# MP-ReID/mp-reid

Measured on AMD Instinct MI355X. Metric: gallery images/s encode + distmat+rerank ms, 20k×20k; mAP/Rank-1 parity, higher is better.
Workload: dtype f16 pairs hi+lo (3 MFMA products per multiply-add, f32-grade), f32 acc; distmat f32 exact; 1 GPU; Market-1501 configs[1]: do_inference ViT-B/16 3368q+15913g/GPU, no rerank; HBM-resident loader; encoder_batch=508, encoder_precision=split, encoder_streams=2, rerank=False, distance_mode=exact

## Files before the change

mp-reid_amd/csrc/gemm_f16.h:

```cpp
#pragma once
#include "common.h"

typedef _Float16 f16x8 __attribute__((ext_vector_type(8)));
typedef float f32x4 __attribute__((ext_vector_type(4)));

constexpr int GBM = 128, GBN = 128, GBK = 64;
constexpr int G_TILE_BYTES = GBM * GBK * 2;
constexpr int G_STAGE_BYTES = 2 * G_TILE_BYTES;
constexpr int G_LDS_BYTES = 2 * G_STAGE_BYTES;
constexpr int BBM = 256, BBN = 256, BBK = 32, B_NSTAGE = 4;
constexpr int B_PART_BYTES = BBM * BBK * 2;
constexpr int B_STAGE_BYTES = 2 * B_PART_BYTES;
constexpr int B_LDS_BYTES = B_NSTAGE * B_STAGE_BYTES;
constexpr int B_LDS_TOTAL = B_LDS_BYTES + 8 * 4096;
constexpr int PBM = 256, PBN = 128, PBK = 32, P_NSTAGE = 3;
constexpr int P_A_BYTES = PBM * PBK * 2;
constexpr int P_B_BYTES = PBN * PBK * 2;
constexpr int P_STAGE_BYTES = P_A_BYTES + P_B_BYTES;
constexpr int P_RING_BYTES = P_NSTAGE * P_STAGE_BYTES;
constexpr int P_LDS_BYTES = P_RING_BYTES + 4 * 1024;

enum GemmEpi {
    GE_F32 = 0,
    GE_BIAS_F16 = 1,
    GE_BIAS_RES = 2,
    GE_BIAS_GELU = 3,
    GE_PATCH = 4,
    GE_EUCLID = 5,
    GE_COSINE = 6,
    GE_BIAS_RELU = 7,
    GE_BIAS_ADD_RELU = 8,
    GE_CAND = 9,
    GE_S_BIAS_F32 = 10,
    GE_S_BIAS_RES = 11,
    GE_S_BIAS_GELU = 12,
    GE_S_PATCH = 13,
    GE_S_BIAS_RELU_PAIR = 14
    , GE_S_BIAS_RES_PAIR = 15
};
constexpr bool gemm_epi_is_split(int epi) { return epi >= GE_S_BIAS_F32 && epi <= GE_S_BIAS_RES_PAIR; }
constexpr bool gemm_epi_has_big(int epi) {
    return epi == GE_F32 || epi == GE_BIAS_F16 || epi == GE_BIAS_RES || epi == GE_BIAS_GELU || epi == GE_EUCLID || epi == GE_PATCH ||
           epi == GE_BIAS_RELU || epi == GE_BIAS_ADD_RELU || epi == GE_CAND || gemm_epi_is_split(epi);
}

struct GemmArgs {
    const _Float16 *A;
    const _Float16 *W;
    int M, N, K;
    int kseg;
    float oscale;
    void *out;
    int64_t ldo;
    const float *bias;
    const float *aux;
    const float *aux2;
    int m_valid, n_valid;
    int P, L;
    const _Float16 *identity;
    const float *rscale;
    const float *cscale;
    const float *tlo, *thi;
    unsigned *cnt_lo, *cnt_hi;
    uint2 *list_lo, *list_hi;
    int cap_lo, cap_hi, sym;
    int stagger;
    int stagger_mode;
    int walk;
    int pair_c;
    _Float16 *pair_out;
    int relu_x;
    unsigned long long *stamps;
};

int launch_gemm_f16(const GemmArgs &a, int epi, hipStream_t stream);
```

mp-reid_amd/csrc/gemm_f16.hip:

```cpp
#include <algorithm>
#include <cstdlib>
#include <type_traits>

#include "gemm_plan.h"

typedef __attribute__((address_space(3))) void lds_ptr_t;
typedef const __attribute__((address_space(1))) void glb_ptr_t;

__device__ __forceinline__ void dma16(const void *gsrc, unsigned char *lds_dst_wave_base) {
    __builtin_amdgcn_global_load_lds((glb_ptr_t *)gsrc, (lds_ptr_t *)lds_dst_wave_base, 16, 0, 0);
}

__device__ __forceinline__ unsigned lds_addr(const void *p) {
    return (unsigned)(uintptr_t)(const __attribute__((address_space(3))) void *)p;
}
__device__ __forceinline__ void dma16_sv(uint64_t sbase, unsigned voff, unsigned lds_dst) {
    unsigned keep;
    asm volatile("s_mov_b32 %0, m0\n\t"
                 "s_mov_b32 m0, %3\n\t"
                 "s_nop 0\n\t"
                 "global_load_lds_dwordx4 %2, %1 nt\n\t"
                 "s_mov_b32 m0, %0"
                 : "=&s"(keep)
                 : "s"(sbase), "v"(voff), "s"(lds_dst)
                 : "memory");
}
__device__ __forceinline__ void store16_sv(uint64_t sbase, unsigned voff, const f32x4 &v) {
    asm volatile("global_store_dwordx4 %0, %1, %2\n\ts_nop 1" ::"v"(voff), "v"(v), "s"(sbase) : "memory");
}
typedef unsigned u32x2 __attribute__((ext_vector_type(2)));
__device__ __forceinline__ void store8_sv(uint64_t sbase, unsigned voff, const u32x2 &v) {
    asm volatile("global_store_dwordx2 %0, %1, %2\n\ts_nop 1" ::"v"(voff), "v"(v), "s"(sbase) : "memory");
}
__device__ __forceinline__ void store16_nt_sv(uint64_t sbase, unsigned voff, const f32x4 &v) {
    asm volatile("global_store_dwordx4 %0, %1, %2 nt\n\ts_nop 1" ::"v"(voff), "v"(v), "s"(sbase) : "memory");
}
template <int F>
__device__ __forceinline__ void store16_flav_sv(uint64_t sbase, unsigned voff, const f32x4 &v) {
    if constexpr (F == 1) asm volatile("global_store_dwordx4 %0, %1, %2\n\ts_nop 1" ::"v"(voff), "v"(v), "s"(sbase) : "memory");
    else if constexpr (F == 2) asm volatile("global_store_dwordx4 %0, %1, %2 sc1\n\ts_nop 1" ::"v"(voff), "v"(v), "s"(sbase) : "memory");
    else if constexpr (F == 3) asm volatile("global_store_dwordx4 %0, %1, %2 sc0 sc1\n\ts_nop 1" ::"v"(voff), "v"(v), "s"(sbase) : "memory");
    else if constexpr (F == 4) asm volatile("global_store_dwordx4 %0, %1, %2 sc0 sc1 nt\n\ts_nop 1" ::"v"(voff), "v"(v), "s"(sbase) : "memory");
    else if constexpr (F == 5) asm volatile("global_store_dwordx4 %0, %1, %2 sc0\n\ts_nop 1" ::"v"(voff), "v"(v), "s"(sbase) : "memory");
    else store16_nt_sv(sbase, voff, v);
}

__device__ __forceinline__ void wait_vmcnt(int n) {
    switch (n) {
    case 12: asm volatile("s_waitcnt vmcnt(12)" ::: "memory"); break;
    case 16: asm volatile("s_waitcnt vmcnt(16)" ::: "memory"); break;
    case 20: asm volatile("s_waitcnt vmcnt(20)" ::: "memory"); break;
    case 24: asm volatile("s_waitcnt vmcnt(24)" ::: "memory"); break;
    case 36: asm volatile("s_waitcnt vmcnt(36)" ::: "memory"); break;
    case 40: asm volatile("s_waitcnt vmcnt(40)" ::: "memory"); break;
    case 44: asm volatile("s_waitcnt vmcnt(44)" ::: "memory"); break;
    case 48: asm volatile("s_waitcnt vmcnt(48)" ::: "memory"); break;
    default: asm volatile("s_waitcnt vmcnt(0)" ::: "memory"); break;
    }
}

__device__ __forceinline__ float quick_gelu(float h) {
    return h * __builtin_amdgcn_rcpf(1.0f + __builtin_amdgcn_exp2f(-1.702f * 1.44269504088896340736f * h));
}

typedef unsigned u32x4_t __attribute__((ext_vector_type(4)));
typedef float f32x4_t __attribute__((ext_vector_type(4)));
__device__ __forceinline__ void store_nt(void *p, const uint4 &v) {
    const u32x4_t nv = {v.x, v.y, v.z, v.w};
    __builtin_nontemporal_store(nv, reinterpret_cast<u32x4_t *>(p));
}
__device__ __forceinline__ void store_nt(float *p, const float4 &v) {
    const f32x4_t nv = {v.x, v.y, v.z, v.w};
    __builtin_nontemporal_store(nv, reinterpret_cast<f32x4_t *>(p));
}

template <int EPI>
__global__ __launch_bounds__(256, 2) void gemm_f16_kernel(GemmArgs g, int tiles_m, int tiles_n) {
    extern __shared__ __attribute__((aligned(16))) unsigned char smem[];

    int tm, tn;
    tile_coords(xcd_remap(blockIdx.x, gridDim.x), tiles_m, tiles_n, 8, tm, tn);
    const int m0 = tm * GBM, n0 = tn * GBN;
    const int tid = threadIdx.x, lane = tid & 63;
    const int wave = __builtin_amdgcn_readfirstlane(tid >> 6);
    const int wm = wave >> 1, wn = wave & 1;
    const int K = g.K;
    constexpr bool SPLIT = gemm_epi_is_split(EPI);
    const int nseg = SPLIT ? g.kseg / GBK : 0;

    const int srow = lane >> 3;
    const int gchunk = (lane & 7) ^ srow;
    const _Float16 *a_src = g.A + (int64_t)(m0 + wave * 32 + srow) * K + gchunk * 8;
    const _Float16 *b_src = g.W + (int64_t)(n0 + wave * 32 + srow) * K + gchunk * 8;
    auto stage = [&](int s, int kt) {
        unsigned char *abase = smem + s * G_STAGE_BYTES + wave * 4096;
        unsigned char *bbase = abase + G_TILE_BYTES;
        const int koff = kt * GBK;
#pragma unroll
        for (int t = 0; t < 4; ++t) {
            dma16(a_src + (int64_t)t * 8 * K + koff, abase + t * 1024);
            dma16(b_src + (int64_t)t * 8 * K + koff, bbase + t * 1024);
        }
    };

    const int frow = lane & 15, fq = lane >> 4;
    const int a_row_off = (wm * 64 + frow) * 128;
    const int b_row_off = (wn * 64 + frow) * 128;
    int ksw[2];
    ksw[0] = ((0 + fq) ^ (lane & 7)) << 4;
    ksw[1] = ((4 + fq) ^ (lane & 7)) << 4;

    f32x4 acc[4][4];
#pragma unroll
    for (int i = 0; i < 4; ++i)
#pragma unroll
        for (int j = 0; j < 4; ++j) acc[i][j] = f32x4{0.f, 0.f, 0.f, 0.f};

    auto compute = [&](int s) {
        const unsigned char *at = smem + s * G_STAGE_BYTES;
        const unsigned char *bt = at + G_TILE_BYTES;
#pragma unroll
        for (int ks = 0; ks < 2; ++ks) {
            f16x8 af[4], bf[4];
#pragma unroll
            for (int i = 0; i < 4; ++i) af[i] = *reinterpret_cast<const f16x8 *>(at + a_row_off + i * 2048 + ksw[ks]);
#pragma unroll
            for (int j = 0; j < 4; ++j) bf[j] = *reinterpret_cast<const f16x8 *>(bt + b_row_off + j * 2048 + ksw[ks]);
#pragma unroll
            for (int i = 0; i < 4; ++i)
#pragma unroll
                for (int j = 0; j < 4; ++j)
                    acc[i][j] = __builtin_amdgcn_mfma_f32_16x16x32_f16(af[i], bf[j], acc[i][j], 0, 0, 0);
        }
    };

    if constexpr (SPLIT) {
        for (int kb = 0; kb < nseg; ++kb) {
            if (kb) __syncthreads();
            {
                unsigned char *abase = smem + wave * 4096;
#pragma unroll
                for (int part = 0; part < 2; ++part) {
                    const int koff = part * g.kseg + kb * GBK;
#pragma unroll
                    for (int t = 0; t < 4; ++t) {
                        dma16(a_src + (int64_t)t * 8 * K + koff, abase + part * G_STAGE_BYTES + t * 1024);
                        dma16(b_src + (int64_t)t * 8 * K + koff, abase + part * G_STAGE_BYTES + G_TILE_BYTES + t * 1024);
                    }
                }
            }
            __syncthreads();
            const unsigned char *ah = smem, *bh = smem + G_TILE_BYTES, *al = smem + G_STAGE_BYTES,
                                *bl = smem + G_STAGE_BYTES + G_TILE_BYTES;
#pragma unroll
            for (int ks = 0; ks < 2; ++ks) {
                f16x8 afh[4], afl[4], bfh[4], bfl[4];
#pragma unroll
                for (int i = 0; i < 4; ++i) {
                    afh[i] = *reinterpret_cast<const f16x8 *>(ah + a_row_off + i * 2048 + ksw[ks]);
                    afl[i] = *reinterpret_cast<const f16x8 *>(al + a_row_off + i * 2048 + ksw[ks]);
                }
#pragma unroll
                for (int j = 0; j < 4; ++j) {
                    bfh[j] = *reinterpret_cast<const f16x8 *>(bh + b_row_off + j * 2048 + ksw[ks]);
                    bfl[j] = *reinterpret_cast<const f16x8 *>(bl + b_row_off + j * 2048 + ksw[ks]);
                }
#pragma unroll
                for (int i = 0; i < 4; ++i)
#pragma unroll
                    for (int j = 0; j < 4; ++j) {
                        acc[i][j] = __builtin_amdgcn_mfma_f32_16x16x32_f16(afh[i], bfh[j], acc[i][j], 0, 0, 0);
                        acc[i][j] = __builtin_amdgcn_mfma_f32_16x16x32_f16(afl[i], bfh[j], acc[i][j], 0, 0, 0);
                        acc[i][j] = __builtin_amdgcn_mfma_f32_16x16x32_f16(afh[i], bfl[j], acc[i][j], 0, 0, 0);
                    }
// ... 154 lines not shown
                    }
                    o[0] = x.x + o[0];
                    o[1] = x.y + o[1];
                    o[2] = x.z + o[2];
                    o[3] = x.w + o[3];
                }
                *reinterpret_cast<float4 *>(dst) = make_float4(o[0], o[1], o[2], o[3]);
                if constexpr (EPI == GE_S_BIAS_RES_PAIR) {
                    typedef _Float16 h4p __attribute__((ext_vector_type(4)));
                    h4p hi, lo;
                    {
                        const float y[4] = {o[0] < 0.f ? 0.f : o[0], o[1] < 0.f ? 0.f : o[1], o[2] < 0.f ? 0.f : o[2],
                                            o[3] < 0.f ? 0.f : o[3]};
                        split_pairs<4>(y, hi, lo);
                    }
                    _Float16 *po = g.pair_out + m * 2 * g.pair_c + nbase + c4;
                    *reinterpret_cast<h4p *>(po) = hi;
                    *reinterpret_cast<h4p *>(po + g.pair_c) = lo;
                }
            }
            __syncthreads();
        }
    } else if constexpr (EPI == GE_BIAS_RES || EPI == GE_EUCLID || EPI == GE_F32) {
        __syncthreads();
        float *wreg = reinterpret_cast<float *>(smem) + wave * (32 * 68);
        float *outp = reinterpret_cast<float *>(g.out);
        const bool vec_ok = (g.ldo % 4 == 0) && ((reinterpret_cast<uintptr_t>(outp) & 15) == 0);
#pragma unroll
        for (int half = 0; half < 2; ++half) {
#pragma unroll
            for (int ii = 0; ii < 2; ++ii)
#pragma unroll
                for (int j = 0; j < 4; ++j)
#pragma unroll
                    for (int r = 0; r < 4; ++r)
                        wreg[(ii * 16 + fq * 4 + r) * 68 + j * 16 + frow] = acc[half * 2 + ii][j][r];
            __syncthreads();
            const int mbase = m0 + wm * 64 + half * 32, nbase = n0 + wn * 64;
            if (vec_ok) {
                const int c4 = (lane & 15) * 4;
                float4 bias4 = make_float4(0.f, 0.f, 0.f, 0.f), bn4 = bias4;
                if (EPI == GE_BIAS_RES) bias4 = *reinterpret_cast<const float4 *>(g.bias + nbase + c4);
                if (EPI == GE_EUCLID) {
                    bn4.x = (nbase + c4 + 0 < g.n_valid) ? g.aux2[nbase + c4 + 0] : 0.f;
                    bn4.y = (nbase + c4 + 1 < g.n_valid) ? g.aux2[nbase + c4 + 1] : 0.f;
                    bn4.z = (nbase + c4 + 2 < g.n_valid) ? g.aux2[nbase + c4 + 2] : 0.f;
                    bn4.w = (nbase + c4 + 3 < g.n_valid) ? g.aux2[nbase + c4 + 3] : 0.f;
                }
#pragma unroll
                for (int it = 0; it < 8; ++it) {
                    const int lr = it * 4 + (lane >> 4);
                    const int m = mbase + lr;
                    const float4 a = *reinterpret_cast<const float4 *>(wreg + lr * 68 + c4);
                    float *dst = outp + (int64_t)m * g.ldo + nbase + c4;
                    if (EPI == GE_F32) {
                        *reinterpret_cast<float4 *>(dst) = a;
                    } else if (EPI == GE_BIAS_RES) {
                        float4 x = *reinterpret_cast<const float4 *>(dst);
                        x.x = x.x + (a.x + bias4.x);
                        x.y = x.y + (a.y + bias4.y);
                        x.z = x.z + (a.z + bias4.z);
                        x.w = x.w + (a.w + bias4.w);
                        *reinterpret_cast<float4 *>(dst) = x;
                    } else {
                        if (m < g.m_valid) {
                            const float am = g.aux[m];
                            float4 o, s4 = make_float4(1.f, 1.f, 1.f, 1.f);
                            if (g.rscale) {
                                const float rs = g.rscale[m];
                                s4 = make_float4(rs * g.cscale[nbase + c4 + 0], rs * g.cscale[nbase + c4 + 1],
                                                 rs * g.cscale[nbase + c4 + 2], rs * g.cscale[nbase + c4 + 3]);
                            }
                            o.x = fmaf(-2.0f, a.x * s4.x, am + bn4.x);
                            o.y = fmaf(-2.0f, a.y * s4.y, am + bn4.y);
                            o.z = fmaf(-2.0f, a.z * s4.z, am + bn4.z);
                            o.w = fmaf(-2.0f, a.w * s4.w, am + bn4.w);
                            if (nbase + c4 + 3 < g.n_valid) {
                                *reinterpret_cast<float4 *>(dst) = o;
                            } else {
                                if (nbase + c4 + 0 < g.n_valid) dst[0] = o.x;
                                if (nbase + c4 + 1 < g.n_valid) dst[1] = o.y;
                                if (nbase + c4 + 2 < g.n_valid) dst[2] = o.z;
                            }
                        }
                    }
                }
            } else {
                const int n = nbase + lane;
                float bias = 0.f, bnv = 0.f;
                if (EPI == GE_BIAS_RES) bias = g.bias[n];
                if (EPI == GE_EUCLID) bnv = (n < g.n_valid) ? g.aux2[n] : 0.f;
#pragma unroll 4
                for (int lr = 0; lr < 32; ++lr) {
                    const int m = mbase + lr;
                    const float a = wreg[lr * 68 + lane];
                    float *dst = outp + (int64_t)m * g.ldo + n;
                    if (EPI == GE_F32) {
                        *dst = a;
                    } else if (EPI == GE_BIAS_RES) {
                        *dst = *dst + (a + bias);
                    } else if (m < g.m_valid && n < g.n_valid) {
                        const float sc = g.rscale ? g.rscale[m] * g.cscale[n] : 1.0f;
                        *dst = fmaf(-2.0f, a * sc, g.aux[m] + bnv);
                    }
                }
            }
            __syncthreads();
        }
    } else {
#pragma unroll
        for (int j = 0; j < 4; ++j) {
            const int n = n0 + wn * 64 + j * 16 + frow;
            float bnv = 0.f;
            if (EPI == GE_COSINE) bnv = (n < g.n_valid) ? g.aux2[n] : 0.f;
#pragma unroll
            for (int i = 0; i < 4; ++i)
#pragma unroll
                for (int r = 0; r < 4; ++r) {
                    const int m = m0 + wm * 64 + i * 16 + fq * 4 + r;
                    const float a = (EPI == GE_S_PATCH) ? acc[i][j][r] * g.oscale : acc[i][j][r];
                    if (EPI == GE_PATCH || EPI == GE_S_PATCH) {
                        if (m < g.m_valid) {
                            const int b = m / g.P, p = m - b * g.P;
                            reinterpret_cast<float *>(g.out)[((int64_t)b * g.L + 1 + p) * g.ldo + n] =
                                a + g.aux[(int64_t)(1 + p) * g.N + n];
                        }
                    } else if (EPI == GE_COSINE) {
                        if (m < g.m_valid && n < g.n_valid) {
                            const float sc = g.rscale ? g.rscale[m] * g.cscale[n] : 1.0f;
                            float c = (a * sc) * __fdiv_rn(1.0f, g.aux[m] * bnv);
                            const float lo = (float)(-1.0 + 0.00001), hi = (float)(1.0 - 0.00001);
                            c = c < lo ? lo : (c > hi ? hi : c);
                            reinterpret_cast<float *>(g.out)[(int64_t)m * g.ldo + n] = acosf(c);
                        }
                    }
                }
        }
    }
}


template <int EPI, int DBG = 0, bool SYM = false>
__global__ __launch_bounds__(512) void gemm_f16_big_kernel(GemmArgs g, int tiles_m, int tiles_n) {
    extern __shared__ __attribute__((aligned(16))) unsigned char smem[];
    const int tid = threadIdx.x, lane = tid & 63;
    const int wave = __builtin_amdgcn_readfirstlane(tid >> 6);
    const int wr = wave >> 2, wc = wave & 3;
    const int K = g.K;
    constexpr bool SPLIT = gemm_epi_is_split(EPI);
    constexpr bool SYM_STORE = (EPI == GE_EUCLID) && SYM;
    constexpr bool SYM_EPI = (EPI == GE_CAND) || SYM_STORE;
    const int nseg = SPLIT ? g.kseg / BBK : 0;
    const int nst = SPLIT ? 3 * nseg : K / BBK;
    auto koff_a = [&](int st) -> int {
        if constexpr (!SPLIT) return st * BBK;
        const int r = st / 3, sidx = st - 3 * r;
        return sidx == 0 ? r * BBK : (sidx == 1 ? g.kseg + r * BBK : -1);
    };
    auto koff_b = [&](int st) -> int {
        if constexpr (!SPLIT) return st * BBK;
        const int r = st / 3, sidx = st - 3 * r;
        return sidx == 0 ? r * BBK : (sidx == 2 ? g.kseg + r * BBK : -1);
    };

    const int ntiles = tiles_m * tiles_n;
    const int nb = (int)gridDim.x;
    const int GR = ((g.walk & 7) == 3 || (g.walk & 8)) ? 4 : ((g.walk & 7) == 4 ? 16 : 8);
    const bool colfast = (g.walk & 7) == 1;
    const int ngroups = (tiles_m + GR - 1) / GR;
    const bool owned = (nb % 8 == 0) && (tiles_m % (8 * GR) == 0 || (ngroups >= 24 && !(g.walk & 16) && !(SYM_EPI && g.sym)));
    const bool blocked = !owned && (nb % 64 == 0) && ntiles >= nb;
    const int xcd = (int)(blockIdx.x & 7), per_xcd = nb >> 3, per_group = GR * tiles_n;
    const int bc_w = per_xcd >> 3;
    const int nbc = blocked ? (tiles_n + bc_w - 1) / bc_w : 1, nbr = (tiles_m + 7) >> 3;
    const bool symc = SYM_EPI && blocked && g.sym != 0;
    int pos = (owned || symc) ? (int)(blockIdx.x >> 3) : (blocked ? 0 : (int)blockIdx.x);
    const int pos_step = (owned || symc) ? per_xcd : (blocked ? 1 : nb);
    int sy_p = 0, sy_cum = 0;
    auto sym_tile_at = [&](int k) -> int {
        for (;;) {
            int b = sy_p * 8 + xcd, br = 0, bcol = 0;
            for (;; ++br) {
                if (br >= nbr) return -1;
                int fb = (br * 8 - bc_w + 1 + bc_w - 1) / bc_w;
                fb = fb < 0 ? 0 : fb;
                const int cnt = nbc - fb;
                if (cnt > 0 && b < cnt) {
                    bcol = fb + b;
                    break;
                }
                b -= cnt > 0 ? cnt : 0;
            }
            const int c_lo = bcol * bc_w, c_hi = min(tiles_n, c_lo + bc_w);
            int cnt = 0;
            for (int r = 0; r < 8; ++r) {
                const int tm = br * 8 + r;
                if (tm < tiles_m) cnt += max(0, c_hi - max(tm, c_lo));
            }
            if (k < sy_cum + cnt) {
                int want = k - sy_cum;
                for (int sl = 0; sl < 8 * bc_w; ++sl) {
                    const int tm = br * 8 + (sl & 7), tn = c_lo + (sl >> 3);
                    if (tm < tiles_m && tn < tiles_n && tn >= tm && want-- == 0) return tm * tiles_n + tn;
                }
            }
            sy_cum += cnt;
            ++sy_p;
        }
    };
    auto tile_at_raw = [&](int p) -> int {
        if (blocked) {
            int b = p * 8 + xcd, br, bcol;
            if (SYM_EPI && g.sym) {
                br = 0;
                for (;; ++br) {
                    if (br >= nbr) return -1;
                    int fb = (br * 8 - bc_w + 1 + bc_w - 1) / bc_w;
                    fb = fb < 0 ? 0 : fb;
                    const int cnt = nbc - fb;
                    if (cnt > 0 && b < cnt) {
                        bcol = fb + b;
                        break;
                    }
                    b -= cnt > 0 ? cnt : 0;
                }
            } else {
                br = b / nbc;
                bcol = b - br * nbc;
            }
            if (br >= nbr) return -1;
            const int slot = (int)(blockIdx.x >> 3);
            const int tm = br * 8 + (slot & 7), tn = bcol * bc_w + (slot >> 3);
            if (SYM_EPI && g.sym && tn < tm) return -2;
            return (tm < tiles_m && tn < tiles_n) ? tm * tiles_n + tn : -2;
        }
        if (!owned) {
            if (p >= ntiles) return -1;
            if (SYM_EPI && g.sym) {
                int tm, tn;
                tile_coords((unsigned)p, tiles_m, tiles_n, 8, tm, tn);
                if (tn < tm) return -2;
            }
            return p;
        }
        const int grp = xcd + 8 * (p / per_group);
        if (grp >= ngroups) return -1;
        const int within = p % per_group;
        const int wrow = colfast ? within / tiles_n : within % GR, wcol = colfast ? within % tiles_n : within / GR;
        if (grp * GR + wrow >= tiles_m) return -2;
        if (SYM_EPI && g.sym && wcol < grp * GR + wrow) return -2;
        return (grp * GR + wrow) * tiles_n + wcol;
    };
    auto tile_at = [&](int &p) -> int {
        if constexpr (SYM_EPI) {
            if (symc) return sym_tile_at(p);
        }
        int t = tile_at_raw(p);
        while (t == -2) {
            p += pos_step;
            t = tile_at_raw(p);
        }
        return t;
    };

    const int drow = lane >> 2;
    const int dchunk = (lane & 3) ^ (((drow >> 3) & 1) * 3);
    const _Float16 *a_src = nullptr, *b_src = nullptr;
    int m0 = 0, n0 = 0;
    auto set_tile = [&](int tile) {
        int tm, tn;
        if (owned || blocked) {
            tm = tile / tiles_n;
            tn = tile - tm * tiles_n;
        } else {
            tile_coords((unsigned)tile, tiles_m, tiles_n, 8, tm, tn);
        }
        m0 = tm * BBM;
        n0 = tn * BBN;
        const int ma = (DBG == 64) ? (tm & 1) * BBM : m0, na = (DBG == 64) ? (tn & 1) * BBN : n0;
        a_src = g.A + (int64_t)(ma + wave * 32 + drow) * K + dchunk * 8;
        b_src = g.W + (int64_t)(na + wave * 32 + drow) * K + dchunk * 8;
    };
    auto dma_stage = [&](int st) {
        unsigned char *abase = smem + (st & (B_NSTAGE - 1)) * B_STAGE_BYTES + wave * 2048;
        unsigned char *bbase = abase + B_PART_BYTES;
        const int koff = koff_a(st), koffb = koff_b(st);
        if (!SPLIT || koff >= 0) {
            dma16(a_src + koff, abase);
            dma16(a_src + (int64_t)16 * K + koff, abase + 1024);
        }
        if (!SPLIT || koffb >= 0) {
            dma16(b_src + koffb, bbase);
            dma16(b_src + (int64_t)16 * K + koffb, bbase + 1024);
        }
    };
    constexpr bool PAIR = !SPLIT && !(DBG & 16);
    auto dma_pair = [&](int st) {
        unsigned char *a0 = smem + (st & (B_NSTAGE - 1)) * B_STAGE_BYTES + wave * 2048;
        unsigned char *a1 = smem + ((st + 1) & (B_NSTAGE - 1)) * B_STAGE_BYTES + wave * 2048;
        const int k0 = st * BBK, k1 = k0 + BBK;
        dma16(a_src + k0, a0);
        dma16(a_src + k1, a1);
        dma16(a_src + (int64_t)16 * K + k0, a0 + 1024);
        dma16(a_src + (int64_t)16 * K + k1, a1 + 1024);
        dma16(b_src + k0, a0 + B_PART_BYTES);
        dma16(b_src + k1, a1 + B_PART_BYTES);
        dma16(b_src + (int64_t)16 * K + k0, a0 + B_PART_BYTES + 1024);
        dma16(b_src + (int64_t)16 * K + k1, a1 + B_PART_BYTES + 1024);
    };
    auto dma_prologue = [&]() {
        if constexpr (PAIR) {
            dma_pair(0);
            if (2 < nst) dma_pair(2);
        } else {
            dma_stage(0);
            if (1 < nst) dma_stage(1);
            if (2 < nst) dma_stage(2);
        }
    };

    const int frow = lane & 15, fq = lane >> 4;
    const int fsw = (fq ^ (((lane >> 3) & 1) * 3)) << 4;
    const int a_off = (wr * 128 + frow) * 64 + fsw;
    const int b_off = B_PART_BYTES + (wc * 64 + frow) * 64 + fsw;
    auto load_frags = [&](int st, f16x8 (&fa)[8], f16x8 (&fb)[4]) {
        const unsigned char *sb = smem + (st & (B_NSTAGE - 1)) * B_STAGE_BYTES;
#pragma unroll
        for (int j = 0; j < 4; ++j) fb[j] = *reinterpret_cast<const f16x8 *>(sb + b_off + j * 1024);
#pragma unroll
        for (int i = 0; i < 8; ++i) fa[i] = *reinterpret_cast<const f16x8 *>(sb + a_off + i * 1024);
    };

    constexpr int CL_CAP = 336;
    int cl_n = 0;
    unsigned *cl_row = reinterpret_cast<unsigned *>(smem + B_LDS_BYTES + wave * 4096);
    unsigned *cl_col = cl_row + CL_CAP;
    unsigned *cl_d = cl_col + CL_CAP;
    auto cl_flush = [&]() {
        if constexpr (EPI == GE_CAND) {
            __builtin_amdgcn_fence(__ATOMIC_RELEASE, "wavefront");
            __builtin_amdgcn_wave_barrier();
            __builtin_amdgcn_fence(__ATOMIC_ACQUIRE, "wavefront");
            for (int e = lane; e < cl_n; e += 64) {
                const unsigned rw = cl_row[e], cw = cl_col[e], dv = cl_d[e];
                const unsigned fl = rw >> 28, row = rw & 0x0fffffffu;
                if (fl & 1u) {
                    const unsigned p = atomicAdd(&g.cnt_lo[row], 1u);
                    if (p < (unsigned)g.cap_lo) g.list_lo[(size_t)row * g.cap_lo + p] = make_uint2(cw, dv);
                }
                if (fl & 2u) {
                    const unsigned p = atomicAdd(&g.cnt_hi[row], 1u);
                    if (p < (unsigned)g.cap_hi) g.list_hi[(size_t)row * g.cap_hi + p] = make_uint2(cw, dv);
                }
                if (fl & 4u) {
                    const unsigned p = atomicAdd(&g.cnt_lo[cw], 1u);
                    if (p < (unsigned)g.cap_lo) g.list_lo[(size_t)cw * g.cap_lo + p] = make_uint2(row, dv);
                }
                if (fl & 8u) {
                    const unsigned p = atomicAdd(&g.cnt_hi[cw], 1u);
                    if (p < (unsigned)g.cap_hi) g.list_hi[(size_t)cw * g.cap_hi + p] = make_uint2(row, dv);
                }
            }
            __builtin_amdgcn_wave_barrier();
            cl_n = 0;
        }
    };

    int tile = tile_at(pos);
    if (tile < 0) return;
    if (g.stagger > 0) {
        const unsigned long long t0 = __builtin_amdgcn_s_memrealtime();
        const unsigned long long wait = g.stagger_mode ? (unsigned long long)g.stagger * ((blockIdx.x >> 3) & 7u) / 8u
                                                       : (unsigned long long)g.stagger * (blockIdx.x & 255u) / 256u;
        while (__builtin_amdgcn_s_memrealtime() - t0 < wait) __builtin_amdgcn_s_sleep(32);
    }
    set_tile(tile);
    dma_prologue();
    [[maybe_unused]] int stamp_tile = 0;
    for (;;) {
    f32x4 acc[8][4];
#pragma unroll
    for (int i = 0; i < 8; ++i)
#pragma unroll
        for (int j = 0; j < 4; ++j) acc[i][j] = f32x4{0.f, 0.f, 0.f, 0.f};

    if constexpr (SPLIT) asm volatile("s_waitcnt vmcnt(4)\n\ts_barrier" ::: "memory");
    else if constexpr (PAIR) {
        if (nst > 2) asm volatile("s_waitcnt vmcnt(8)\n\ts_barrier" ::: "memory");
        else asm volatile("s_waitcnt vmcnt(0)\n\ts_barrier" ::: "memory");
    } else if (nst > 2) asm volatile("s_waitcnt vmcnt(8)\n\ts_barrier" ::: "memory");
    else asm volatile("s_waitcnt vmcnt(4)\n\ts_barrier" ::: "memory");

    auto stamp = [&](int which) {
        if constexpr ((DBG & 32) != 0) {
            if (g.stamps && tid == 0 && stamp_tile < 32)
                g.stamps[((size_t)blockIdx.x * 32 + stamp_tile) * 8 + which] = __builtin_amdgcn_s_memrealtime();
        }
    };
    stamp(0);
    f16x8 fa0[8], fb0[4], fa1[8], fb1[4];
    load_frags(0, fa0, fb0);

    auto mfma32 = [&](f16x8 (&fa)[8], f16x8 (&fb)[4]) {
#pragma unroll
        for (int i = 0; i < 8; ++i)
#pragma unroll
            for (int j = 0; j < 4; ++j)
                acc[i][j] = __builtin_amdgcn_mfma_f32_16x16x32_f16(fa[i], fb[j], acc[i][j], 0, 0, 0);
    };
    auto step_steady = [&](auto ODD_, int t, f16x8 (&fa)[8], f16x8 (&fb)[4], f16x8 (&na)[8], f16x8 (&nb)[4]) {
        constexpr bool ODD = decltype(ODD_)::value != 0;
        constexpr bool ISSUE = !PAIR || ODD;
        if constexpr (!PAIR) asm volatile("s_waitcnt vmcnt(4)\n\ts_barrier" ::: "memory");
        else if constexpr (ODD) asm volatile("s_waitcnt vmcnt(1) lgkmcnt(0)\n\ts_barrier" ::: "memory");
        else asm volatile("s_waitcnt vmcnt(8)\n\ts_barrier" ::: "memory");
        unsigned char *dbase = smem + ((t + 3) & (B_NSTAGE - 1)) * B_STAGE_BYTES + wave * 2048;
        unsigned char *dbase2 = smem + ((t + 4) & (B_NSTAGE - 1)) * B_STAGE_BYTES + wave * 2048;
        const unsigned char *sb = smem + ((t + 1) & (B_NSTAGE - 1)) * B_STAGE_BYTES;
        const int koff = koff_a(t + 3), koffb = koff_b(t + 3);
#define MPREID_FRAG_B(j) nb[j] = *reinterpret_cast<const f16x8 *>(sb + b_off + (j) * 1024)
#define MPREID_FRAG_A(i) na[i] = *reinterpret_cast<const f16x8 *>(sb + a_off + (i) * 1024)
#define MPREID_MFMA_ROWS(i0)                                                                             \
    _Pragma("unroll") for (int ii = (i0); ii < (i0) + 2; ++ii) _Pragma("unroll") for (int j = 0; j < 4; ++j) { \
        if constexpr (!(DBG & 2))                                                                        \
            acc[ii][j] = __builtin_amdgcn_mfma_f32_16x16x32_f16(fa[ii], fb[j], acc[ii][j], 0, 0, 0);       \
        else                                                                                             \
            asm volatile("" ::"v"(fa[ii]), "v"(fb[j]));                                                  \
    }
        if constexpr (!(DBG & 1) && ISSUE) {
            dma16(a_src + koff, dbase);
            if constexpr (PAIR) dma16(a_src + koff + BBK, dbase2);
        }
        if constexpr (!(DBG & 4)) { MPREID_FRAG_B(0); MPREID_FRAG_B(1); MPREID_FRAG_B(2); }
        MPREID_MFMA_ROWS(0);
        __builtin_amdgcn_sched_barrier(0);
        if constexpr (!(DBG & 1) && ISSUE) {
            dma16(a_src + (int64_t)16 * K + koff, dbase + 1024);
            if constexpr (PAIR) dma16(a_src + (int64_t)16 * K + koff + BBK, dbase2 + 1024);
        }
        if constexpr (!(DBG & 4)) { MPREID_FRAG_B(3); MPREID_FRAG_A(0); MPREID_FRAG_A(1); }
        MPREID_MFMA_ROWS(2);
        __builtin_amdgcn_sched_barrier(0);
        if constexpr (!(DBG & 1) && ISSUE) {
            dma16(b_src + koffb, dbase + B_PART_BYTES);
            if constexpr (PAIR) dma16(b_src + koffb + BBK, dbase2 + B_PART_BYTES);
        }
        if constexpr (!(DBG & 4)) { MPREID_FRAG_A(2); MPREID_FRAG_A(3); MPREID_FRAG_A(4); }
        MPREID_MFMA_ROWS(4);
        __builtin_amdgcn_sched_barrier(0);
        if constexpr (!(DBG & 1) && ISSUE) {
            dma16(b_src + (int64_t)16 * K + koffb, dbase + B_PART_BYTES + 1024);
            if constexpr (PAIR) dma16(b_src + (int64_t)16 * K + koffb + BBK, dbase2 + B_PART_BYTES + 1024);
        }
        if constexpr (!(DBG & 4)) { MPREID_FRAG_A(5); MPREID_FRAG_A(6); MPREID_FRAG_A(7); }
        MPREID_MFMA_ROWS(6);
        __builtin_amdgcn_sched_barrier(0);
#undef MPREID_FRAG_A
#undef MPREID_FRAG_B
#undef MPREID_MFMA_ROWS
    };
    auto step_tail = [&](int t, f16x8 (&fa)[8], f16x8 (&fb)[4], f16x8 (&na)[8], f16x8 (&nb)[4]) {
        if (t + 1 < nst) {
            if constexpr (PAIR) {
                if (!(t & 1) && t + 3 < nst) asm volatile("s_waitcnt vmcnt(8)\n\ts_barrier" ::: "memory");
                else asm volatile("s_waitcnt vmcnt(0)\n\ts_barrier" ::: "memory");
            } else {
                if (t + 2 < nst) asm volatile("s_waitcnt vmcnt(4)\n\ts_barrier" ::: "memory");
                else asm volatile("s_waitcnt vmcnt(0)\n\ts_barrier" ::: "memory");
                if (t + 3 < nst) dma_stage(t + 3);
            }
            load_frags(t + 1, na, nb);
        }
        mfma32(fa, fb);
    };
    if constexpr (SPLIT) {
        auto sstep = [&](auto S_, auto TAIL_, int t) {
            constexpr int S = decltype(S_)::value;
            constexpr bool TAIL = decltype(TAIL_)::value;
            constexpr int s0 = S % 3;
            constexpr bool ldA = s0 != 1, ldB = s0 != 0;
            constexpr bool dmA = s0 != 2, dmB = s0 != 1;
            f16x8 (&fa)[8] = (S & 1) ? fa1 : fa0;
            f16x8 (&fb)[4] = (s0 == 2) ? fb1 : fb0;
            f16x8 (&na)[8] = (S < 3) ? fa1 : fa0;
            f16x8 (&nb)[4] = (s0 == 1) ? fb1 : fb0;
            constexpr bool more1 = !TAIL || S < 5, more3 = !TAIL || S < 3;
            if constexpr (more1) {
                if constexpr (TAIL && S >= 4) asm volatile("s_waitcnt vmcnt(0)\n\ts_barrier" ::: "memory");
                else if constexpr (s0 == 1) asm volatile("s_waitcnt vmcnt(4)\n\ts_barrier" ::: "memory");
                else asm volatile("s_waitcnt vmcnt(2)\n\ts_barrier" ::: "memory");
            }
            unsigned char *dbase = smem + ((t + 3) & (B_NSTAGE - 1)) * B_STAGE_BYTES + wave * 2048;
            const unsigned char *sb = smem + ((t + 1) & (B_NSTAGE - 1)) * B_STAGE_BYTES;
            const int r3 = (t + 3) / 3;
            const int koff = (s0 == 1 ? g.kseg : 0) + r3 * BBK, koffb = (s0 == 2 ? g.kseg : 0) + r3 * BBK;
            auto piece = [&](int q) {
                if (!more3) return;
                if (dmA && q < 2) dma16(a_src + (int64_t)(q * 16) * K + koff, dbase + q * 1024);
                else if (dmB && q - (dmA ? 2 : 0) >= 0 && q - (dmA ? 2 : 0) < 2)
                    dma16(b_src + (int64_t)((q - (dmA ? 2 : 0)) * 16) * K + koffb, dbase + B_PART_BYTES + (q - (dmA ? 2 : 0)) * 1024);
            };
            auto rd_a = [&](int i) { if (more1) na[i] = *reinterpret_cast<const f16x8 *>(sb + a_off + i * 1024); };
            auto rd_b = [&](int j) { if (more1) nb[j] = *reinterpret_cast<const f16x8 *>(sb + b_off + j * 1024); };
#pragma unroll
            for (int gq = 0; gq < 4; ++gq) {
                piece(gq);
                if constexpr (ldA && ldB) {
                    if (gq == 0) { rd_b(0); rd_b(1); rd_b(2); }
                    if (gq == 1) { rd_b(3); rd_a(0); rd_a(1); }
                    if (gq == 2) { rd_a(2); rd_a(3); rd_a(4); }
                    if (gq == 3) { rd_a(5); rd_a(6); rd_a(7); }
                } else if constexpr (ldA) {
                    rd_a(2 * gq);
                    rd_a(2 * gq + 1);
                } else {
                    rd_b(gq);
                }
#pragma unroll
                for (int ii = 2 * gq; ii < 2 * gq + 2; ++ii)
#pragma unroll
                    for (int j = 0; j < 4; ++j)
                        acc[ii][j] = __builtin_amdgcn_mfma_f32_16x16x32_f16(fa[ii], fb[j], acc[ii][j], 0, 0, 0);
                __builtin_amdgcn_sched_barrier(0);
            }
        };
        using std::integral_constant;
        int t = 0;
        for (; t + 6 < nst; t += 6) {
            sstep(integral_constant<int, 0>{}, integral_constant<bool, false>{}, t);
            sstep(integral_constant<int, 1>{}, integral_constant<bool, false>{}, t + 1);
            sstep(integral_constant<int, 2>{}, integral_constant<bool, false>{}, t + 2);
            sstep(integral_constant<int, 3>{}, integral_constant<bool, false>{}, t + 3);
            sstep(integral_constant<int, 4>{}, integral_constant<bool, false>{}, t + 4);
            sstep(integral_constant<int, 5>{}, integral_constant<bool, false>{}, t + 5);
        }
        sstep(integral_constant<int, 0>{}, integral_constant<bool, true>{}, t);
        sstep(integral_constant<int, 1>{}, integral_constant<bool, true>{}, t + 1);
        sstep(integral_constant<int, 2>{}, integral_constant<bool, true>{}, t + 2);
        sstep(integral_constant<int, 3>{}, integral_constant<bool, true>{}, t + 3);
        sstep(integral_constant<int, 4>{}, integral_constant<bool, true>{}, t + 4);
        sstep(integral_constant<int, 5>{}, integral_constant<bool, true>{}, t + 5);
    } else {
    int t = 0;
    for (; t + 4 < nst; t += 2) {
        step_steady(std::integral_constant<int, 0>{}, t, fa0, fb0, fa1, fb1);
        step_steady(std::integral_constant<int, 1>{}, t + 1, fa1, fb1, fa0, fb0);
    }
    for (; t < nst; t += 2) {
        step_tail(t, fa0, fb0, fa1, fb1);
        step_tail(t + 1, fa1, fb1, fa0, fb0);
    }
    }

    __syncthreads();
    stamp(1);
    const int cur_m0 = m0, cur_n0 = n0;
    pos += pos_step;
    const int next_tile = tile_at(pos);
    unsigned char *patch = smem + B_LDS_BYTES;
    if constexpr (DBG & 8) {
#pragma unroll
        for (int i = 0; i < 8; ++i)
#pragma unroll
            for (int j = 0; j < 4; ++j) asm volatile("" ::"v"(acc[i][j]));
    } else if constexpr (EPI == GE_CAND) {
        const bool mirror = g.sym != 0 && cur_m0 != cur_n0;
        float *tp = reinterpret_cast<float *>(smem + wave * 16384);
        const int rb = cur_m0 + wr * 128, cb = cur_n0 + wc * 64;
        const float NEG = -__builtin_huge_valf(), POS = __builtin_huge_valf();
        float *rt = tp + 1024;
        float *ct = rt + 384;
        {
            const float a0 = g.aux[rb + lane], a1 = g.aux[rb + 64 + lane];
            const float l0 = g.tlo[rb + lane], l1 = g.tlo[rb + 64 + lane];
            const float h0 = g.thi[rb + lane], h1 = g.thi[rb + 64 + lane];
            const int c = cb + lane;
            const bool cv = c < g.n_valid;
            const float cn = cv ? g.aux2[c] : 0.f;
            const float cl = (mirror && cv) ? g.tlo[c] : NEG, chh = (mirror && cv) ? g.thi[c] : POS;
            rt[lane] = a0; rt[64 + lane] = a1;
            rt[128 + lane] = l0; rt[192 + lane] = l1;
            rt[256 + lane] = h0; rt[320 + lane] = h1;
            ct[lane] = cn; ct[64 + lane] = cl; ct[128 + lane] = chh;
        }
        __builtin_amdgcn_fence(__ATOMIC_RELEASE, "wavefront");
        __builtin_amdgcn_wave_barrier();
        __builtin_amdgcn_fence(__ATOMIC_ACQUIRE, "wavefront");
        float bnv[4], tlc[4], thc[4];
        unsigned cvm = 0u;
#pragma unroll
        for (int j = 0; j < 4; ++j) {
            const int cl_ = j * 16 + frow;
            cvm |= (cb + cl_ < g.n_valid) ? (0xfu << (4 * j)) : 0u;
            bnv[j] = ct[cl_];
            tlc[j] = ct[64 + cl_];
            thc[j] = ct[128 + cl_];
        }
#pragma unroll
        for (int i = 0; i < 8; ++i) {
            const int rl = i * 16 + fq * 4;
            const int r0 = rb + rl;
            const float4 an4 = *reinterpret_cast<const float4 *>(rt + rl);
            const float4 tl4 = *reinterpret_cast<const float4 *>(rt + 128 + rl);
            const float4 th4 = *reinterpret_cast<const float4 *>(rt + 256 + rl);
            const float anr[4] = {an4.x, an4.y, an4.z, an4.w}, tlr[4] = {tl4.x, tl4.y, tl4.z, tl4.w},
                        thr[4] = {th4.x, th4.y, th4.z, th4.w};
            unsigned rvm = 0u;
#pragma unroll
            for (int r = 0; r < 4; ++r) rvm |= (r0 + r < g.m_valid) ? (0x1111u << r) : 0u;
            unsigned hit = 0u;
#pragma unroll
            for (int j = 0; j < 4; ++j)
#pragma unroll
                for (int r = 0; r < 4; ++r) {
                    const float a = acc[i][j][r];
                    tp[(fq * 4 + r) * 64 + j * 16 + frow] = a;
                    const float d = fmaf(-2.0f, a, anr[r] + bnv[j]);
                    const bool h = (d <= tlr[r]) | (d >= thr[r]) | (d <= tlc[j]) | (d >= thc[j]);
                    hit |= h ? (1u << (j * 4 + r)) : 0u;
                }
            hit &= cvm & rvm;
            __builtin_amdgcn_fence(__ATOMIC_RELEASE, "wavefront");
            __builtin_amdgcn_wave_barrier();
            __builtin_amdgcn_fence(__ATOMIC_ACQUIRE, "wavefront");
            unsigned long long bal = __ballot(hit != 0u);
            if (g.stagger & 2) bal = 0;
            while (bal) {
                const int add = __popcll(bal);
                if (cl_n + add > CL_CAP) cl_flush();
                if (hit) {
                    const int e = __ffs((int)hit) - 1;
                    hit &= hit - 1u;
                    const int j = e >> 2, r = e & 3;
                    const float a = tp[(fq * 4 + r) * 64 + j * 16 + frow];
                    const float anx = r == 0 ? anr[0] : (r == 1 ? anr[1] : (r == 2 ? anr[2] : anr[3]));
                    const float tlx = r == 0 ? tlr[0] : (r == 1 ? tlr[1] : (r == 2 ? tlr[2] : tlr[3]));
                    const float thx = r == 0 ? thr[0] : (r == 1 ? thr[1] : (r == 2 ? thr[2] : thr[3]));
                    const float bnx = j == 0 ? bnv[0] : (j == 1 ? bnv[1] : (j == 2 ? bnv[2] : bnv[3]));
                    const float tcx = j == 0 ? tlc[0] : (j == 1 ? tlc[1] : (j == 2 ? tlc[2] : tlc[3]));
                    const float hcx = j == 0 ? thc[0] : (j == 1 ? thc[1] : (j == 2 ? thc[2] : thc[3]));
                    const float d = fmaf(-2.0f, a, anx + bnx);
                    const unsigned fl = (d <= tlx ? 1u : 0u) | (d >= thx ? 2u : 0u) | (d <= tcx ? 4u : 0u) | (d >= hcx ? 8u : 0u);
                    const int p = cl_n + __popcll(bal & ((1ull << lane) - 1ull));
                    cl_row[p] = (unsigned)(r0 + r) | (fl << 28);
                    cl_col[p] = (unsigned)(cb + j * 16 + frow);
                    cl_d[p] = __float_as_uint(d);
                }
                cl_n += add;
                bal = __ballot(hit != 0u);
            }
            __builtin_amdgcn_wave_barrier();
        }
        if (next_tile < 0) cl_flush();
        asm volatile("s_barrier" ::: "memory");
    } else if constexpr (EPI == GE_BIAS_F16 || EPI == GE_BIAS_GELU || EPI == GE_BIAS_RELU) {
        _Float16 *wreg = reinterpret_cast<_Float16 *>(patch + wave * 4096);
        _Float16 *out = reinterpret_cast<_Float16 *>(g.out);
        float bias[4];
#pragma unroll
        for (int j = 0; j < 4; ++j) bias[j] = g.bias[cur_n0 + wc * 64 + j * 16 + frow];
#pragma unroll
        for (int i = 0; i < 8; ++i) {
#pragma unroll
            for (int j = 0; j < 4; ++j)
#pragma unroll
                for (int r = 0; r < 4; ++r) {
                    float v = acc[i][j][r] + bias[j];
                    if (EPI == GE_BIAS_GELU) v = quick_gelu(v);
                    if (EPI == GE_BIAS_RELU) v = v < 0.f ? 0.f : v;
                    wreg[(fq * 4 + r) * 72 + j * 16 + frow] = (_Float16)v;
                }
            __builtin_amdgcn_fence(__ATOMIC_RELEASE, "wavefront");
            __builtin_amdgcn_wave_barrier();
            __builtin_amdgcn_fence(__ATOMIC_ACQUIRE, "wavefront");
#pragma unroll
            for (int it = 0; it < 2; ++it) {
                const int lr = it * 8 + (lane >> 3), ch = lane & 7;
                const uint4 v = *reinterpret_cast<const uint4 *>(wreg + lr * 72 + ch * 8);
                _Float16 *dsth = out + (int64_t)(cur_m0 + wr * 128 + i * 16 + lr) * g.ldo + cur_n0 + wc * 64 + ch * 8;
                if (EPI == GE_BIAS_RELU) *reinterpret_cast<uint4 *>(dsth) = v;
                else store_nt(dsth, v);
            }
            __builtin_amdgcn_wave_barrier();
        }
    } else if constexpr (EPI == GE_S_BIAS_GELU || EPI == GE_S_BIAS_RELU_PAIR) {
        _Float16 *whi = reinterpret_cast<_Float16 *>(patch + wave * 4096);
        _Float16 *wlo = reinterpret_cast<_Float16 *>(smem + wave * 4096);
        _Float16 *out = reinterpret_cast<_Float16 *>(g.out);
        float bias[4];
#pragma unroll
        for (int j = 0; j < 4; ++j) bias[j] = g.bias[cur_n0 + wc * 64 + j * 16 + frow];
#pragma unroll
        for (int i = 0; i < 8; ++i) {
#pragma unroll
// ... 1219 lines not shown
```

Baseline: 17090 images/s.

## Restructure split-precision GEMM LDS ring into two whole k-blocks with scalar-base DMA

The split (hi+lo) GEMM path used to stream three product stages per k-step through a 4-stage ring, loading A and B pieces separately for each stage. It now holds two full k-blocks (A_hi, B_hi, A_lo, B_lo) in the ring and loads the next block in pieces spread across the three MFMA stages. It uses scalar-base plus vector-offset global_load_lds without the nt hint, so the data can stay in cache. The aim is to stop reloading shared hi tiles and to cut per-load address arithmetic, at the cost of a more fragile waitcnt/barrier schedule and a loop that assumes nseg is even.

New measurement: 17220 images/s (median of 6 runs). No clear change (+0.7%).

```diff
diff --git a/mp-reid_amd/csrc/gemm_f16.h b/mp-reid_amd/csrc/gemm_f16.h
--- a/mp-reid_amd/csrc/gemm_f16.h
+++ b/mp-reid_amd/csrc/gemm_f16.h
@@ -12,6 +12,8 @@
 constexpr int B_PART_BYTES = BBM * BBK * 2;
 constexpr int B_STAGE_BYTES = 2 * B_PART_BYTES;
 constexpr int B_LDS_BYTES = B_NSTAGE * B_STAGE_BYTES;
+constexpr int B_KBLOCK_BYTES = 4 * B_PART_BYTES;
+static_assert(2 * B_KBLOCK_BYTES == B_LDS_BYTES, "the split ring holds exactly two k blocks");
 constexpr int B_LDS_TOTAL = B_LDS_BYTES + 8 * 4096;
 constexpr int PBM = 256, PBN = 128, PBK = 32, P_NSTAGE = 3;
 constexpr int P_A_BYTES = PBM * PBK * 2;
diff --git a/mp-reid_amd/csrc/gemm_f16.hip b/mp-reid_amd/csrc/gemm_f16.hip
--- a/mp-reid_amd/csrc/gemm_f16.hip
+++ b/mp-reid_amd/csrc/gemm_f16.hip
@@ -20,6 +20,17 @@
                  "s_mov_b32 m0, %3\n\t"
                  "s_nop 0\n\t"
                  "global_load_lds_dwordx4 %2, %1 nt\n\t"
+                 "s_mov_b32 m0, %0"
+                 : "=&s"(keep)
+                 : "s"(sbase), "v"(voff), "s"(lds_dst)
+                 : "memory");
+}
+__device__ __forceinline__ void dma16_sv_cached(uint64_t sbase, unsigned voff, unsigned lds_dst) {
+    unsigned keep;
+    asm volatile("s_mov_b32 %0, m0\n\t"
+                 "s_mov_b32 m0, %3\n\t"
+                 "s_nop 0\n\t"
+                 "global_load_lds_dwordx4 %2, %1\n\t"
                  "s_mov_b32 m0, %0"
                  : "=&s"(keep)
                  : "s"(sbase), "v"(voff), "s"(lds_dst)
@@ -480,16 +491,6 @@
     constexpr bool SYM_EPI = (EPI == GE_CAND) || SYM_STORE;
     const int nseg = SPLIT ? g.kseg / BBK : 0;
     const int nst = SPLIT ? 3 * nseg : K / BBK;
-    auto koff_a = [&](int st) -> int {
-        if constexpr (!SPLIT) return st * BBK;
-        const int r = st / 3, sidx = st - 3 * r;
-        return sidx == 0 ? r * BBK : (sidx == 1 ? g.kseg + r * BBK : -1);
-    };
-    auto koff_b = [&](int st) -> int {
-        if constexpr (!SPLIT) return st * BBK;
-        const int r = st / 3, sidx = st - 3 * r;
-        return sidx == 0 ? r * BBK : (sidx == 2 ? g.kseg + r * BBK : -1);
-    };
 
     const int ntiles = tiles_m * tiles_n;
     const int nb = (int)gridDim.x;
@@ -594,6 +595,7 @@
     const int drow = lane >> 2;
     const int dchunk = (lane & 3) ^ (((drow >> 3) & 1) * 3);
     const _Float16 *a_src = nullptr, *b_src = nullptr;
+    [[maybe_unused]] uint64_t a_sbase = 0, b_sbase = 0;
     int m0 = 0, n0 = 0;
     auto set_tile = [&](int tile) {
         int tm, tn;
@@ -606,21 +608,34 @@
         m0 = tm * BBM;
         n0 = tn * BBN;
         const int ma = (DBG == 64) ? (tm & 1) * BBM : m0, na = (DBG == 64) ? (tn & 1) * BBN : n0;
-        a_src = g.A + (int64_t)(ma + wave * 32 + drow) * K + dchunk * 8;
-        b_src = g.W + (int64_t)(na + wave * 32 + drow) * K + dchunk * 8;
+        if constexpr (SPLIT) {
+            a_sbase = reinterpret_cast<uint64_t>(g.A + (int64_t)(ma + wave * 32) * K);
+            b_sbase = reinterpret_cast<uint64_t>(g.W + (int64_t)(na + wave * 32) * K);
+        } else {
+            a_src = g.A + (int64_t)(ma + wave * 32 + drow) * K + dchunk * 8;
+            b_src = g.W + (int64_t)(na + wave * 32 + drow) * K + dchunk * 8;
+        }
     };
     auto dma_stage = [&](int st) {
         unsigned char *abase = smem + (st & (B_NSTAGE - 1)) * B_STAGE_BYTES + wave * 2048;
         unsigned char *bbase = abase + B_PART_BYTES;
-        const int koff = koff_a(st), koffb = koff_b(st);
-        if (!SPLIT || koff >= 0) {
-            dma16(a_src + koff, abase);
-            dma16(a_src + (int64_t)16 * K + koff, abase + 1024);
-        }
-        if (!SPLIT || koffb >= 0) {
-            dma16(b_src + koffb, bbase);
-            dma16(b_src + (int64_t)16 * K + koffb, bbase + 1024);
-        }
+        const int koff = st * BBK;
+        dma16(a_src + koff, abase);
+        dma16(a_src + (int64_t)16 * K + koff, abase + 1024);
+        dma16(b_src + koff, bbase);
+        dma16(b_src + (int64_t)16 * K + koff, bbase + 1024);
+    };
+    const unsigned dma_voff = (unsigned)(drow * K + dchunk * 8) * 2u;
+    const unsigned ring_lds = __builtin_amdgcn_readfirstlane(lds_addr(smem)) + wave * 2048;
+    auto dma_kpiece = [&](int r, int slot, int q) {
+        const int part = q >> 1, half = q & 1;
+        const uint64_t sbase = ((part & 1) ? b_sbase : a_sbase) +
+                               (uint64_t)(((int64_t)(half * 16) * K + (part >= 2 ? g.kseg : 0) + r * BBK) * 2);
+        dma16_sv_cached(sbase, dma_voff, ring_lds + slot * B_KBLOCK_BYTES + part * B_PART_BYTES + half * 1024);
+    };
+    auto dma_kblock = [&](int r) {
+#pragma unroll
+        for (int q = 0; q < 8; ++q) dma_kpiece(r, r & 1, q);
     };
     constexpr bool PAIR = !SPLIT && !(DBG & 16);
     auto dma_pair = [&](int st) {
@@ -637,7 +652,9 @@
         dma16(b_src + (int64_t)16 * K + k1, a1 + B_PART_BYTES + 1024);
     };
     auto dma_prologue = [&]() {
-        if constexpr (PAIR) {
+        if constexpr (SPLIT) {
+            dma_kblock(0);
+        } else if constexpr (PAIR) {
             dma_pair(0);
             if (2 < nst) dma_pair(2);
         } else {
@@ -745,7 +762,7 @@
         unsigned char *dbase = smem + ((t + 3) & (B_NSTAGE - 1)) * B_STAGE_BYTES + wave * 2048;
         unsigned char *dbase2 = smem + ((t + 4) & (B_NSTAGE - 1)) * B_STAGE_BYTES + wave * 2048;
         const unsigned char *sb = smem + ((t + 1) & (B_NSTAGE - 1)) * B_STAGE_BYTES;
-        const int koff = koff_a(t + 3), koffb = koff_b(t + 3);
+        const int koff = (t + 3) * BBK, koffb = koff;
 #define MPREID_FRAG_B(j) nb[j] = *reinterpret_cast<const f16x8 *>(sb + b_off + (j) * 1024)
 #define MPREID_FRAG_A(i) na[i] = *reinterpret_cast<const f16x8 *>(sb + a_off + (i) * 1024)
 #define MPREID_MFMA_ROWS(i0)                                                                             \
@@ -802,34 +819,33 @@
         mfma32(fa, fb);
     };
     if constexpr (SPLIT) {
-        auto sstep = [&](auto S_, auto TAIL_, int t) {
+        auto sstep = [&](auto S_, auto TAIL_, int r) {
             constexpr int S = decltype(S_)::value;
             constexpr bool TAIL = decltype(TAIL_)::value;
             constexpr int s0 = S % 3;
             constexpr bool ldA = s0 != 1, ldB = s0 != 0;
-            constexpr bool dmA = s0 != 2, dmB = s0 != 1;
             f16x8 (&fa)[8] = (S & 1) ? fa1 : fa0;
             f16x8 (&fb)[4] = (s0 == 2) ? fb1 : fb0;
             f16x8 (&na)[8] = (S < 3) ? fa1 : fa0;
             f16x8 (&nb)[4] = (s0 == 1) ? fb1 : fb0;
-            constexpr bool more1 = !TAIL || S < 5, more3 = !TAIL || S < 3;
+            constexpr bool more1 = !TAIL || S < 5;
+            constexpr int cur = S / 3;
+            constexpr int nxt = (s0 == 2) ? (cur ^ 1) : cur;
+            constexpr bool more3 = !TAIL || S < 3;
             if constexpr (more1) {
                 if constexpr (TAIL && S >= 4) asm volatile("s_waitcnt vmcnt(0)\n\ts_barrier" ::: "memory");
                 else if constexpr (s0 == 1) asm volatile("s_waitcnt vmcnt(4)\n\ts_barrier" ::: "memory");
                 else asm volatile("s_waitcnt vmcnt(2)\n\ts_barrier" ::: "memory");
             }
-            unsigned char *dbase = smem + ((t + 3) & (B_NSTAGE - 1)) * B_STAGE_BYTES + wave * 2048;
-            const unsigned char *sb = smem + ((t + 1) & (B_NSTAGE - 1)) * B_STAGE_BYTES;
-            const int r3 = (t + 3) / 3;
-            const int koff = (s0 == 1 ? g.kseg : 0) + r3 * BBK, koffb = (s0 == 2 ? g.kseg : 0) + r3 * BBK;
-            auto piece = [&](int q) {
-                if (!more3) return;
-                if (dmA && q < 2) dma16(a_src + (int64_t)(q * 16) * K + koff, dbase + q * 1024);
-                else if (dmB && q - (dmA ? 2 : 0) >= 0 && q - (dmA ? 2 : 0) < 2)
-                    dma16(b_src + (int64_t)((q - (dmA ? 2 : 0)) * 16) * K + koffb, dbase + B_PART_BYTES + (q - (dmA ? 2 : 0)) * 1024);
+            auto piece = [&](int gq) {
+                if constexpr (more3) {
+                    if (gq < (s0 == 0 ? 4 : 2)) dma_kpiece(r + cur + 1, cur ^ 1, (s0 == 0 ? 0 : (s0 == 1 ? 4 : 6)) + gq);
+                }
             };
-            auto rd_a = [&](int i) { if (more1) na[i] = *reinterpret_cast<const f16x8 *>(sb + a_off + i * 1024); };
-            auto rd_b = [&](int j) { if (more1) nb[j] = *reinterpret_cast<const f16x8 *>(sb + b_off + j * 1024); };
+            const unsigned char *sa = smem + nxt * B_KBLOCK_BYTES + (s0 == 0 ? 2 * B_PART_BYTES : 0);
+            const unsigned char *sw = smem + nxt * B_KBLOCK_BYTES + (s0 == 1 ? 2 * B_PART_BYTES : 0);
+            auto rd_a = [&](int i) { if (more1) na[i] = *reinterpret_cast<const f16x8 *>(sa + a_off + i * 1024); };
+            auto rd_b = [&](int j) { if (more1) nb[j] = *reinterpret_cast<const f16x8 *>(sw + b_off + j * 1024); };
 #pragma unroll
             for (int gq = 0; gq < 4; ++gq) {
                 piece(gq);
@@ -853,21 +869,21 @@
             }
         };
         using std::integral_constant;
-        int t = 0;
-        for (; t + 6 < nst; t += 6) {
-            sstep(integral_constant<int, 0>{}, integral_constant<bool, false>{}, t);
-            sstep(integral_constant<int, 1>{}, integral_constant<bool, false>{}, t + 1);
-            sstep(integral_constant<int, 2>{}, integral_constant<bool, false>{}, t + 2);
-            sstep(integral_constant<int, 3>{}, integral_constant<bool, false>{}, t + 3);
-            sstep(integral_constant<int, 4>{}, integral_constant<bool, false>{}, t + 4);
-            sstep(integral_constant<int, 5>{}, integral_constant<bool, false>{}, t + 5);
-        }
-        sstep(integral_constant<int, 0>{}, integral_constant<bool, true>{}, t);
-        sstep(integral_constant<int, 1>{}, integral_constant<bool, true>{}, t + 1);
-        sstep(integral_constant<int, 2>{}, integral_constant<bool, true>{}, t + 2);
-        sstep(integral_constant<int, 3>{}, integral_constant<bool, true>{}, t + 3);
-        sstep(integral_constant<int, 4>{}, integral_constant<bool, true>{}, t + 4);
-        sstep(integral_constant<int, 5>{}, integral_constant<bool, true>{}, t + 5);
+        int r = 0;
+        for (; r + 2 < nseg; r += 2) {
+            sstep(integral_constant<int, 0>{}, integral_constant<bool, false>{}, r);
+            sstep(integral_constant<int, 1>{}, integral_constant<bool, false>{}, r);
+            sstep(integral_constant<int, 2>{}, integral_constant<bool, false>{}, r);
+            sstep(integral_constant<int, 3>{}, integral_constant<bool, false>{}, r);
+            sstep(integral_constant<int, 4>{}, integral_constant<bool, false>{}, r);
+            sstep(integral_constant<int, 5>{}, integral_constant<bool, false>{}, r);
+        }
+        sstep(integral_constant<int, 0>{}, integral_constant<bool, true>{}, r);
+        sstep(integral_constant<int, 1>{}, integral_constant<bool, true>{}, r);
+        sstep(integral_constant<int, 2>{}, integral_constant<bool, true>{}, r);
+        sstep(integral_constant<int, 3>{}, integral_constant<bool, true>{}, r);
+        sstep(integral_constant<int, 4>{}, integral_constant<bool, true>{}, r);
+        sstep(integral_constant<int, 5>{}, integral_constant<bool, true>{}, r);
     } else {
     int t = 0;
     for (; t + 4 < nst; t += 2) {
```
